# GolosChain/language-detector

Measured on AMD Instinct MI355X. Metric: docs/sec, higher is better.
Workload: dtype u8

## Files before the change

language-detector_amd/csrc/cld_wave.hip:

```cpp

namespace cld {
namespace wave {


__device__ __forceinline__ int ufl(int v) { return __builtin_amdgcn_readfirstlane(v); }
__device__ __forceinline__ uint32_t uflu(uint32_t v) { return (uint32_t)__builtin_amdgcn_readfirstlane((int)v); }
__device__ __forceinline__ uint64_t ufl64(uint64_t v) {
  return ((uint64_t)uflu((uint32_t)(v >> 32)) << 32) | uflu((uint32_t)v);
}
__device__ __forceinline__ int rdl(int v, int l) { return __builtin_amdgcn_readlane(v, l); }
__device__ __forceinline__ uint32_t rdlu(uint32_t v, int l) { return (uint32_t)__builtin_amdgcn_readlane((int)v, l); }
__device__ __forceinline__ uint64_t rdl64(uint64_t v, int l) {
  return ((uint64_t)rdlu((uint32_t)(v >> 32), l) << 32) | rdlu((uint32_t)v, l);
}


__device__ __forceinline__ void wsync() {
  __builtin_amdgcn_fence(__ATOMIC_RELEASE, "wavefront");
  __builtin_amdgcn_wave_barrier();
  __builtin_amdgcn_fence(__ATOMIC_ACQUIRE, "wavefront");
}

__device__ __forceinline__ uint64_t lanemask_lt(int lane) { return lane ? (~0ull >> (64 - lane)) : 0ull; }
__device__ __forceinline__ int below(uint64_t m) {
  return (int)__builtin_amdgcn_mbcnt_hi((uint32_t)(m >> 32), __builtin_amdgcn_mbcnt_lo((uint32_t)m, 0u));
}
__device__ __forceinline__ int lane_here() {
  int l;
  asm volatile("v_mbcnt_lo_u32_b32 %0, -1, 0\n\tv_mbcnt_hi_u32_b32 %0, -1, %0" : "=v"(l));
  return l;
}

template <int N, class V>
__device__ __forceinline__ V pick(const V (&a)[N], int r) {
  V v = a[0];
#pragma unroll
  for (int i = 1; i < N; ++i) if (r == i) v = a[i];
  return v;
}
template <int N, class V>
__device__ __forceinline__ void put_lane(V (&a)[N], int r, int l, V val) {
  const bool me = (int)__lane_id() == l;
#pragma unroll
  for (int i = 0; i < N; ++i)
    if (r == i && me) a[i] = val;
}
template <int N>
__device__ __forceinline__ void or_bit(uint64_t (&a)[N], int r, int l) {
#pragma unroll
  for (int i = 0; i < N; ++i) if (r == i) a[i] |= 1ull << l;
}

constexpr int kDppRowShr = 0x110, kDppRowBcast15 = 0x142, kDppRowBcast31 = 0x143;
template <class Op>
__device__ __forceinline__ uint32_t dpp_scan_incl(uint32_t x, uint32_t id, Op op) {
  const int xi = (int)x;
  x = op(x, (uint32_t)__builtin_amdgcn_update_dpp((int)id, xi, kDppRowShr | 1, 0xF, 0xF, false));
  x = op(x, (uint32_t)__builtin_amdgcn_update_dpp((int)id, (int)x, kDppRowShr | 2, 0xF, 0xF, false));
  x = op(x, (uint32_t)__builtin_amdgcn_update_dpp((int)id, (int)x, kDppRowShr | 4, 0xF, 0xF, false));
  x = op(x, (uint32_t)__builtin_amdgcn_update_dpp((int)id, (int)x, kDppRowShr | 8, 0xF, 0xF, false));
  x = op(x, (uint32_t)__builtin_amdgcn_update_dpp((int)id, (int)x, kDppRowBcast15, 0xA, 0xF, false));
  x = op(x, (uint32_t)__builtin_amdgcn_update_dpp((int)id, (int)x, kDppRowBcast31, 0xC, 0xF, false));
  return x;
}
struct OpAdd { __device__ uint32_t operator()(uint32_t a, uint32_t b) const { return a + b; } };
struct OpMax { __device__ uint32_t operator()(uint32_t a, uint32_t b) const { return a > b ? a : b; } };
struct OpMin { __device__ uint32_t operator()(uint32_t a, uint32_t b) const { return a < b ? a : b; } };
struct OpOr { __device__ uint32_t operator()(uint32_t a, uint32_t b) const { return a | b; } };

constexpr int kDppWaveShr1 = 0x138, kDppWaveShl1 = 0x130;
__device__ __forceinline__ uint32_t wshr1(uint32_t x, uint32_t first) {
  return (uint32_t)__builtin_amdgcn_update_dpp((int)first, (int)x, kDppWaveShr1, 0xF, 0xF, false);
}
__device__ __forceinline__ uint64_t wshr1_64(uint64_t x) {
  return ((uint64_t)wshr1((uint32_t)(x >> 32), (uint32_t)(x >> 32)) << 32) | wshr1((uint32_t)x, (uint32_t)x);
}

__device__ __forceinline__ int excl_scan(int v, int lane) {
  (void)lane;
  return (int)dpp_scan_incl((uint32_t)v, 0u, OpAdd()) - v;
}
__device__ __forceinline__ int wsum(int v) { return rdl((int)dpp_scan_incl((uint32_t)v, 0u, OpAdd()), 63); }
__device__ __forceinline__ uint32_t wmax(uint32_t v) { return rdlu(dpp_scan_incl(v, 0u, OpMax()), 63); }
__device__ __forceinline__ uint32_t wmin(uint32_t v) { return rdlu(dpp_scan_incl(v, 0xFFFFFFFFu, OpMin()), 63); }
__device__ __forceinline__ uint64_t wor64(uint64_t v) {
  const uint32_t lo = rdlu(dpp_scan_incl((uint32_t)v, 0u, OpOr()), 63);
  const uint32_t hi = rdlu(dpp_scan_incl((uint32_t)(v >> 32), 0u, OpOr()), 63);
  return ((uint64_t)hi << 32) | lo;
}

template <int CAP>
struct Cfg {
  static constexpr int DOC = CAP + 32;
  static constexpr int NM = (CAP + 63) / 64;
  static constexpr int SB = CAP + 72;
  static constexpr int LB = (SB * 3) / 2 + 64;
  static constexpr int NR = 2;
  static constexpr int NB = NR * 64;
  static constexpr int QM = ((LB + 63) / 64) * 2;
  static constexpr int NE = 160;
  static constexpr int ND = 96;
  static constexpr int NX = 160;
  static constexpr int MAXCH = NE / kChunksizeQuads + 3;
  static_assert(NB < kMaxScoringHits - 1, "a round must never reach the reference's hit cap");
  static_assert(CAP < 2048, "spans of a short document can never reach the squeeze test");
  static_assert((NE + ND + NX + 9) * kMaxLgProbScore < 65536, "tote headroom");
};

template <int CAP>
struct Smem {
  using C = Cfg<CAP>;
  uint8_t doc[C::DOC];
  uint8_t sn[C::DOC];
  uint64_t lsm[C::NM];
  uint64_t ent[C::NM];
  union alignas(16) {
    uint8_t sbuf[C::SB];
    uint16_t wsp[C::NB + 1];
    struct {
      int32_t theta[C::MAXCH];
      uint16_t st[3][C::MAXCH + 1];
    };
  };
  union alignas(16) {
    uint8_t lbuf[C::LB];
    uint32_t tote[128];
  };
  union alignas(16) {
    uint16_t nx[CAP];
    uint32_t low[CAP];
    struct {
      uint32_t be_lp[C::NE];
      uint16_t be_off[C::NE + 1];
    } e;
  } a;
  union alignas(16) {
    struct {
      uint16_t d_off[C::ND]; uint32_t d_ind[C::ND];
      uint16_t x_off[C::NX]; uint32_t x_ind[C::NX];
    };
    struct {
      uint32_t qmark[C::QM];
      uint16_t qchn[C::NB];
      uint16_t nxq[C::LB];
    };
  };
  uint16_t E[C::MAXCH];
  uint32_t lo[C::MAXCH];
  uint32_t ring[2][4];
  DocTote dt;
};

template <int NM>
__device__ __forceinline__ int find_first(const uint64_t* m, int from, int L) {
  if (from >= L) return L;
  int w = from >> 6;
  uint64_t x = ufl64(m[w]) & (~0ull << (from & 63));
  for (;;) {
    if (x) { int r = (w << 6) + __builtin_ctzll(x); return r < L ? r : L; }
    ++w;
    if (w >= NM || (w << 6) >= L) return L;
    x = ufl64(m[w]);
  }
}

__device__ __forceinline__ int cpt_index(uint32_t b0, uint32_t b1, uint32_t b2, int n) {
  if (n == 1) return (int)b0;
  if (n == 2) return 128 + (int)((b0 & 0x1F) << 6 | (b1 & 0x3F));
  return 2176 + (int)((b0 & 0x0F) << 12 | (b1 & 0x3F) << 6 | (b2 & 0x3F));
}

__device__ __forceinline__ uint32_t pack_lowered(uint64_t e) {
  const uint32_t olen = (uint32_t)(e >> 11) & 15;
  return (((e >> 10) & 1) && olen <= 3) ? (((uint32_t)(e >> 32) & 0xFFFFFFu) | olen << 24) : 0xFFFFFFFFu;
}

template <int CAP, bool PLAIN>
__device__ bool load_document(const DevTables& T, const uint8_t* __restrict__ g, int L, Smem<CAP>& s, int lane,
                              const uint8_t* __restrict__ hf, bool& lowv) {
  if constexpr (PLAIN) hf = nullptr;
  lowv = false;
  using C = Cfg<CAP>;
  static_assert(CAP == 256 && C::DOC == 288, "one aligned dword per lane covers the document");
// ... 3 lines not shown
    const uint32_t* gw = reinterpret_cast<const uint32_t*>(ga - (uintptr_t)sh);
    const int nw = (L + sh + 3) >> 2;
    const uint32_t w0 = lane < nw ? gld(gw + lane) : 0u;
    const uint32_t w64 = nw > 64 ? gld(gw + 64) : 0u;
    const uint32_t nxt = (uint32_t)__builtin_amdgcn_update_dpp((int)w64, (int)w0, kDppWaveShl1, 0xF, 0xF, false);
    const uint32_t v = sh == 0 ? w0 : __builtin_amdgcn_alignbyte(nxt, w0, (uint32_t)sh);
    const int nb = L - 4 * lane;
    const uint32_t keep = nb >= 4 ? 0xFFFFFFFFu : nb <= 0 ? 0u : (1u << (8 * nb)) - 1u;
    reinterpret_cast<uint32_t*>(s.doc)[lane] = v & keep;
    if (lane < (C::DOC - 256) / 4) reinterpret_cast<uint32_t*>(s.doc)[64 + lane] = 0u;
    if (hf) {
      for (int w = 0; w < C::NM; ++w) {
        const uint64_t m = __ballot(w * 64 + lane < L && gld(hf + w * 64 + lane) != 0);
        if (lane == 0) s.ent[w] = m;
      }
    } else if (!PLAIN && lane < C::NM) {
      s.ent[lane] = 0ull;
    }
  }
  wsync();
  DocView dv{s.doc, L};
  {
    int slow = 0, conts = 0, need = 0;
    int idx[C::NM];
#pragma unroll
    for (int w = 0; w < C::NM; ++w) idx[w] = -1;
#pragma unroll
    for (int w = 0; w < C::NM; ++w) {
      if (w * 64 >= L) break;
      const int p = w * 64 + lane;
      const uint32_t c = s.doc[p], b1 = s.doc[p + 1], b2 = s.doc[p + 2];
      const bool in = p < L;
      const bool cont = in && (c & 0xC0) == 0x80, lead = in && !cont;
      const int n = utf8_len((uint8_t)c);
      const bool bad = lead && (n > 3 || p + n > L || (n >= 2 && (b1 & 0xC0) != 0x80) || (n == 3 && (b2 & 0xC0) != 0x80));
      conts += cont ? 1 : 0;
      slow |= bad ? 1 : 0;
      const bool ok = lead && !bad;
      need += ok ? n - 1 : 0;
      idx[w] = ok ? cpt_index(c, b1, b2, n) : -1;
    }
    uint64_t ev[C::NM];
#pragma unroll
    for (int w = 0; w < C::NM; ++w) ev[w] = idx[w] >= 0 ? gld(T.cpt + idx[w]) : 0ull;
#pragma unroll
    for (int w = 0; w < C::NM; ++w) {
      if (w * 64 >= L) break;
      const int p = w * 64 + lane;
      const uint64_t e = ev[w];
      const int st = (int)((e >> 8) & 3);
      slow |= st == 3 ? 1 : 0;
      s.sn[p] = (uint8_t)e;
      s.a.low[p] = pack_lowered(e);
      const uint64_t m = __ballot(st == 1 && (e & 0xFF) != 0);
      if (lane == 0) s.lsm[w] = m;
    }
    slow |= wsum(conts - need) != 0 ? 1 : 0;
    if (__ballot(slow != 0) == 0) {
      if (lane < 4) s.sn[L + lane] = (uint8_t)script_num(T, dv, L + lane);
      wsync();
      lowv = true;
      return true;
    }
  }
  for (int p = lane; p < L + 4; p += 64) s.sn[p] = (uint8_t)script_num(T, dv, p);
  for (int p = lane; p < L; p += 64) s.a.nx[p] = (uint16_t)(p + scan_to_letter_or_special(T, dv, p, L - p));
  wsync();
  int bad = 0, conts = 0, need = 0;
  for (int p = lane; p < L; p += 64) {
    uint8_t c = s.doc[p];
    if ((c & 0xC0) == 0x80) { ++conts; continue; }
    int n = utf8_len(c);
    if (p + n > L) { bad = 1; continue; }
    for (int k = 1; k < n; ++k) bad |= ((s.doc[p + k] & 0xC0) != 0x80);
    need += n - 1;
    int np = s.a.nx[p];
    if (np != p) {
      int q = p + n;
      int want = q >= L ? L : (int)s.a.nx[q];
      bad |= (np != want);
    }
  }
  bad |= (wsum(conts) != wsum(need)) ? 1 : 0;
  if (__ballot(bad != 0)) return false;
  for (int w = 0; w < C::NM; ++w) {
    int p = w * 64 + lane;
    bool ls = false;
    if (p < L) ls = ((s.doc[p] & 0xC0) != 0x80) && s.a.nx[p] == p && s.sn[p] != 0;
    uint64_t m = __ballot(ls);
    if (lane == 0) s.lsm[w] = m;
  }
  wsync();
  return true;
}

template <int CAP>
__device__ bool stale_script_amp(const DevTables& T, Smem<CAP>& s, int L, const uint8_t* __restrict__ hf, int lane) {
  const int common = (int)T.common, inherited = (int)T.inherited;
  int hit = 0;
  for (int x = lane; x < L; x += 64) {
    if (!((s.ent[x >> 6] >> (x & 63)) & 1) || !(gld(hf + x) & 2) || (s.doc[x] & 0xC0) == 0x80) continue;
    const int sc = s.sn[x];
    if (sc == 0 || sc == common) continue;
    int b = x - 1;
    while (b > 0 && (s.doc[b] & 0xC0) == 0x80) --b;
    if (b < 0) continue;
    const int scb = s.sn[b];
    if (scb == 0 || scb == common || scb == inherited) continue;
    int a = b - 1;
    while (a > 0 && (s.doc[a] & 0xC0) == 0x80) --a;
    if (a < 0) continue;
    const int sca = s.sn[a];
    if (sca == 0 || sca == common) continue;
    hit |= (sca == inherited || (scb != sca && sc != sca)) ? 1 : 0;
  }
  return __ballot(hit != 0) != 0;
}

template <int CAP, bool PLAIN>
__device__ int next_span(const DevTables& T, Smem<CAP>& s, int L, int& next, int& ulscript, int lane) {
  lane = lane_here();
  using C = Cfg<CAP>;
  const int common = (int)T.common, inherited = (int)T.inherited;
  const int q = find_first<C::NM>(s.lsm, next, L);
  if (q >= L) { next = L; return 0; }
  const int spanscript = ufl(s.sn[q]);
  ulscript = spanscript;
  if (lane == 0) s.sbuf[0] = ' ';
  int put = 1, take = L;
  bool run = true;
  for (int w = q >> 6; w < C::NM && w * 64 < L; ++w) {
    const int x = w * 64 + lane;
    const bool valid = x >= q && x < L;
    const uint32_t c = valid ? s.doc[x] : 0u;
    const bool lead = valid && (c & 0xC0) != 0x80;
    bool brk = false, ok = false, foreign = false;
    if (lead) {
      const int sc = s.sn[x];
      if (sc != spanscript && sc != inherited) {
        if (sc == common) {
          brk = true;
        } else {
          const int xn = x + utf8_len((uint8_t)c);
          const int sc2 = (!PLAIN && xn < 64 * C::NM && ((s.ent[xn >> 6] >> (xn & 63)) & 1)) ? 0 : s.sn[xn];
          brk = sc2 != common && sc2 != spanscript;
        }
      }
      if ((s.lsm[w] >> lane) & 1) {
        if (sc == spanscript || sc == inherited) ok = true;
        else foreign = true;
      }
    }
    const uint64_t Bm = __ballot(brk), Om = __ballot(ok);
    const uint64_t evm = Bm | Om;
    const uint64_t ev_le = evm & (lane == 63 ? ~0ull : ((2ull << lane) - 1)), ev_lt = evm & lanemask_lt(lane);
    const bool inrun = ev_le ? ((Om >> (63 - __builtin_clzll(ev_le))) & 1) : run;
    const bool prev_run = ev_lt ? ((Om >> (63 - __builtin_clzll(ev_lt))) & 1) : run;
    const uint64_t Em = __ballot(foreign && (brk || !prev_run));
    const int stop = Em ? __builtin_ctzll(Em) : 64;
    const bool cp = valid && inrun && lane < stop;
    const bool sep = brk && prev_run && lane <= stop;
    const int cnt = (cp ? 1 : 0) + (sep ? 1 : 0);
    const int pos = put + excl_scan(cnt, lane);
    if (cp) s.sbuf[pos] = (uint8_t)c;
    if (sep) s.sbuf[pos] = ' ';
    put = rdl(pos + cnt, 63);
    if (stop < 64) {
      take = w * 64 + stop;
      run = false;
      break;
    }
    if (evm) run = (Om >> (63 - __builtin_clzll(evm))) & 1;
  }
  if (run) {
    if (lane == 0) s.sbuf[put] = ' ';
    ++put;
  }
  if (lane < 4) s.sbuf[put + lane] = lane < 3 ? ' ' : 0;
  next = take;
  wsync();
  return put;
}

__device__ __forceinline__ void setb(uint64_t& o, int i, uint32_t v) {
  o = (o & ~(0xFFull << (8 * i))) | ((uint64_t)(v & 0xFF) << (8 * i));
}
template <bool PIN = false>
__device__ bool lower_char_sm(const DevSM& sm_in, const uint8_t* src, int n, uint64_t& out, int& olen) {
  const DevSM sm_pin = PIN ? pinned_sm(sm_in) : DevSM{};
  const DevSM& sm = PIN ? sm_pin : sm_in;
  const int sh = (int)sm.shift;
  const int nE = 1 << sh;
  const int64_t tb0 = sm.state0;
  int64_t tb = tb0;
  out = 0; olen = 0;
  for (int i = 0; i < n; ++i) {
    const uint8_t c = src[i];
    const int e = sm8(sm, tb + c);
    if (olen >= 8) return false;
    out |= (uint64_t)c << (8 * olen);
    ++olen;
    if (e < kExitIllegalStructure) { tb = tb0 + ((int64_t)e << sh); continue; }
    switch (e) {
      case kExitReplace31:
        if (olen < 3) return false;
        olen -= 2; setb(out, olen - 1, sm8(sm, tb + c + nE * 1));
        out &= olen >= 8 ? ~0ull : ((1ull << (8 * olen)) - 1);
        break;
      case kExitReplace32:
        if (olen < 3) return false;
        olen -= 1; setb(out, olen - 2, sm8(sm, tb + c + nE * 2)); setb(out, olen - 1, sm8(sm, tb + c + nE * 1));
        out &= (1ull << (8 * olen)) - 1;
        break;
      case kExitReplace21:
// ... 48 lines not shown
    int m = utf8_len((uint8_t)b);
    if (i + m > olen) return false;
    for (int k = 1; k < m; ++k)
      if ((((uint32_t)(out >> (8 * (i + k)))) & 0xC0) != 0x80) return false;
    i += m;
  }
  return true;
}
__device__ __forceinline__ bool lower_char(const DevTables& T, const uint8_t* src, int n, uint64_t& out, int& olen) {
  return lower_char_sm(T.lower, src, n, out, olen);
}

template <int CAP>
__device__ int lower_span(const DevTables& T, Smem<CAP>& s, int text_bytes, int lane) {
  lane = lane_here();
  using C = Cfg<CAP>;
  const int ilen = text_bytes + 3;
  int obase = 0;
  int bad = 0;
  for (int w0 = 0; w0 < ilen; w0 += 64) {
    const int p = w0 + lane;
    uint64_t o = 0;
    int olen = 0;
    if (p < ilen && (s.sbuf[p] & 0xC0) != 0x80) {
      const int n = utf8_len(s.sbuf[p]);
      const uint32_t b1 = s.sbuf[p + 1], b2 = s.sbuf[p + 2];
      const bool wf = n <= 3 && (n < 2 || (b1 & 0xC0) == 0x80) && (n < 3 || (b2 & 0xC0) == 0x80);
      const uint64_t e = wf ? T.cpt[cpt_index(s.sbuf[p], b1, b2, n)] : 0ull;
      if ((e >> 10) & 1) {
        olen = (int)((e >> 11) & 15);
        o = e >> 32;
      } else if (!lower_char_sm<true>(T.lower, &s.sbuf[p], n, o, olen)) {
        bad = 1;
        olen = 0;
      }
    }
    const int pre = excl_scan(olen, lane);
    const int tot = rdl(pre + olen, 63);
    if (obase + tot + 4 > C::LB - 16) bad = 1;
    else
      for (int k = 0; k < olen; ++k) s.lbuf[obase + pre + k] = (uint8_t)(o >> (8 * k));
    obase += tot;
  }
  if (__ballot(bad != 0)) return -1;
  for (int k = lane; k < 20; k += 64) s.lbuf[obase + k] = 0;
  wsync();
  return obase - 3;
}

template <int CAP, bool PLAIN>
__device__ int span_lowered(const DevTables& T, Smem<CAP>& s, int L, int& next, int& ulscript, int lane, bool lowv) {
  lane = lane_here();
  using C = Cfg<CAP>;
  const int common = (int)T.common, inherited = (int)T.inherited;
  const int q = find_first<C::NM>(s.lsm, next, L);
  if (q >= L) { next = L; return 0; }
  const int spanscript = ufl(s.sn[q]);
  ulscript = spanscript;
  uint32_t ev[C::NM];
  if (lowv) {
#pragma unroll
    for (int w = 0; w < C::NM; ++w) ev[w] = s.a.low[w * 64 + lane];
  } else {
    int idx[C::NM];
#pragma unroll
    for (int w = 0; w < C::NM; ++w) {
      const int p = w * 64 + lane;
      const uint32_t c = s.doc[p], b1 = s.doc[p + 1], b2 = s.doc[p + 2];
      const int n = utf8_len((uint8_t)c);
      const bool wf = p >= q && p < L && (c & 0xC0) != 0x80 && n <= 3 && (n < 2 || (b1 & 0xC0) == 0x80) &&
                      (n < 3 || (b2 & 0xC0) == 0x80);
      idx[w] = wf ? cpt_index(c, b1, b2, n) : -1;
    }
    uint64_t raw[C::NM];
#pragma unroll
    for (int w = 0; w < C::NM; ++w) raw[w] = idx[w] >= 0 ? gld(T.cpt + idx[w]) : 0ull;
#pragma unroll
    for (int w = 0; w < C::NM; ++w) ev[w] = pack_lowered(raw[w]);
  }
  static_assert(C::NM == 4, "four windows");
  uint32_t e0 = ev[0], e1 = ev[1], e2 = ev[2], e3 = ev[3];
  for (int i = q >> 6; i > 0; --i) { e0 = e1; e1 = e2; e2 = e3; }
  if (lane == 0) s.lbuf[0] = ' ';
  int put = 1, take = L, bad = 0;
  bool run = true;
  for (int w = q >> 6; w < C::NM && w * 64 < L; ++w) {
    const int x = w * 64 + lane;
    const bool valid = x >= q && x < L;
    const uint32_t c = valid ? s.doc[x] : 0u;
    const bool lead = valid && (c & 0xC0) != 0x80;
    bool brk = false, ok = false, foreign = false;
    if (lead) {
      const int sc = s.sn[x];
      if (sc != spanscript && sc != inherited) {
        if (sc == common) {
          brk = true;
        } else {
          const int xn = x + utf8_len((uint8_t)c);
          const int sc2 = (!PLAIN && xn < 64 * C::NM && ((s.ent[xn >> 6] >> (xn & 63)) & 1)) ? 0 : s.sn[xn];
          brk = sc2 != common && sc2 != spanscript;
        }
      }
      if ((s.lsm[w] >> lane) & 1) {
        if (sc == spanscript || sc == inherited) ok = true;
        else foreign = true;
      }
    }
    const uint64_t Bm = __ballot(brk), Om = __ballot(ok), Fm = __ballot(foreign), Lm = __ballot(lead);
    const uint64_t evm = Bm | Om;
    const uint64_t ca = Om | ~evm;
    const uint64_t prevm = (ca + Om + (run ? 1ull : 0ull)) ^ ca ^ Om;
    const uint64_t runm = Om | (~evm & prevm);
    const uint64_t Em = Fm & (Bm | ~prevm);
    const int stop = Em ? __builtin_ctzll(Em) : 64;
    const uint64_t lt_stop = Em ? (Em & (0 - Em)) - 1 : ~0ull, le_stop = Em ? (Em ^ (Em - 1)) : ~0ull;
    const bool cl = ((Lm & runm & lt_stop) >> lane) & 1;
    const bool sep = ((Bm & prevm & le_stop) >> lane) & 1;
    const uint32_t e = e0;
    const bool low = e != 0xFFFFFFFFu;
    bad |= (cl && !low) ? 1 : 0;
    const int olen = sep ? 1 : (cl && low) ? (int)(e >> 24) : 0;
    const uint32_t o = sep ? (uint32_t)' ' : e;
    const int pos = put + excl_scan(olen, lane);
    put = rdl(pos + olen, 63);
    if (put + 8 > C::LB - 16) { bad = 1; break; }
    for (int k = 0; k < olen; ++k) s.lbuf[pos + k] = (uint8_t)(o >> (8 * k));
    if (stop < 64) {
      take = w * 64 + stop;
      run = false;
      break;
    }
    run = (runm >> 63) != 0;
    e0 = e1; e1 = e2; e2 = e3;
  }
  if (__ballot(bad != 0)) {
    const int tb = next_span<CAP, PLAIN>(T, s, L, next, ulscript, lane);
    return lower_span<CAP>(T, s, tb, lane);
  }
  if (run) {
    if (lane == 0) s.lbuf[put] = ' ';
    ++put;
  }
  if (lane < 23) s.lbuf[put + lane] = lane < 3 ? ' ' : 0;
  next = take;
  wsync();
  return put;
}

__device__ __forceinline__ uint32_t quad_hash_lds(const uint8_t* text, int p, int n) {
  const uint32_t* tw = reinterpret_cast<const uint32_t*>(text);
  const int i0 = p >> 2;
  const uint32_t sh = (uint32_t)(p & 3);
  const uint32_t x0 = tw[i0], x1 = tw[i0 + 1], x2 = tw[i0 + 2], x3 = tw[i0 + 3];
  const uint32_t y0 = __builtin_amdgcn_alignbyte(x1, x0, sh), y1 = __builtin_amdgcn_alignbyte(x2, x1, sh),
                 y2 = __builtin_amdgcn_alignbyte(x3, x2, sh);
  const uint32_t pre = (text[p - 1] == ' ' ? 0x00004444u : 0u) | (text[p + n] == ' ' ? 0x44440000u : 0u);
  const uint32_t m = (n & 3) ? (1u << (8 * (n & 3))) - 1u : 0xFFFFFFFFu;
  const uint32_t a0 = n <= 4 ? (y0 & m) : y0;
  const uint32_t w0 = (a0 ^ (a0 >> 3)) ^ pre;
  const uint32_t a1 = n <= 8 ? (y1 & m) : y1;
  const uint32_t w1 = a1 ^ (a1 << 4);
  const uint32_t a2 = y2 & m;
  const uint32_t w2 = a2 ^ (a2 << 2);
  const uint32_t r = n <= 4 ? w0 : n <= 8 ? w0 + w1 : w0 + w1 + w2;
  return n == 0 ? 0u : r;
}

template <int CAP>
__device__ __forceinline__ bool emit_base(Smem<CAP>& s, const DevTbl& bo, const DevTbl& bo2, bool kept, uint32_t ind,
                                          int off, int& eb) {
  using C = Cfg<CAP>;
  uint32_t l1 = 0, l2 = 0;
  if (kept) {
    const DevTbl* lb = &bo;
    if (ind & 0x80000000u) { lb = &bo2; ind &= ~0x80000000u; }
    if (ind < lb->size_one) {
      l1 = ind_at(*lb, ind);
    } else {
      ind += ind - lb->size_one;
      l1 = ind_at(*lb, ind); l2 = ind_at(*lb, ind + 1);
      if (l1 == 0) { l1 = l2; l2 = 0; }
    }
  }
  const uint64_t m1 = __ballot(l1 != 0), m2 = __ballot(l2 != 0);
  const int o = eb + below(m1) + below(m2);
  eb += __popcll(m1) + __popcll(m2);
  if (eb > C::NE) return false;
  if (l1) { s.a.e.be_off[o] = (uint16_t)off; s.a.e.be_lp[o] = l1; }
  if (l2) { s.a.e.be_off[o + 1] = (uint16_t)off; s.a.e.be_lp[o + 1] = l2; }
  return true;
}

template <int CAP>
__device__ int quad_hits(const DevTables& T, Smem<CAP>& s, int limit, int& nb, int& eb, int& start, int& nw, int lane) {
  lane = lane_here();
  using C = Cfg<CAP>;
  const uint8_t* text = s.lbuf;
  start = 1;
  if (text[start] == ' ') ++start;
  uint16_t* nfo = s.nxq;
  const int last = start < limit ? limit : start;
  int nws = start < limit ? 1 : 0;
  nw = 0;
  for (int w0 = start; w0 <= last; w0 += 64) {
    const int p = w0 + lane;
    const bool in = p < limit;
    const int pc = p <= last ? p : start;
    const uint32_t c0 = text[pc];
    const int a1 = pc + adv_but_space((uint8_t)c0);
    const int a2 = a1 + adv_but_space(text[a1]);
    const uint32_t c2 = text[a2];
    const int a3 = a2 + adv_but_space((uint8_t)c2);
    const int a4 = a3 + adv_but_space(text[a3]);
    const int nx = a2 + adv_space_vowel((uint8_t)c2);
    const bool fin = text[a4] == ' ' || a2 >= limit || nx >= limit;
    if (in) nfo[p] = (uint16_t)((a4 - p) | ((nx - p) << 5) | (fin ? 0x400 : 0));
    const bool sp = p <= last && c0 == ' ';
    const uint64_t m = __ballot(sp);
    if (sp) {
      const int k = nw + below(m);
      if (k <= C::NB) s.wsp[k] = (uint16_t)p;
    }
    nw += __popcll(m);
    nws += __popcll(__ballot(sp && p < limit - 1));
  }
  if (nws > C::NB || nw > C::NB) return -1;
  if (lane < C::QM) s.qmark[lane] = 0u;
  wsync();
#pragma unroll
  for (int r = 0; r < C::NR; ++r) {
    if (r * 64 >= nws) break;
    const int i = r * 64 + lane;
    if (i < nws) {
      int p = i == 0 ? start : s.wsp[i - 1] + 1;
      for (;;) {
        atomicOr(&s.qmark[p >> 5], 1u << (p & 31));
        const uint32_t f = nfo[p];
        if (f & 0x400) break;
        p += (f >> 5) & 31;
      }
    }
  }
  wsync();
  int n = 0;
  for (int w = start >> 6; w * 64 < limit; ++w) {
    const uint64_t m = ufl64(*reinterpret_cast<const uint64_t*>(&s.qmark[2 * w]));
    if ((m >> lane) & 1) {
      const int k = n + below(m);
      if (k < C::NB) s.qchn[k] = (uint16_t)(w * 64 + lane);
    }
    n += __popcll(m);
  }
  if (n > C::NB) return -1;
  wsync();
  const int end = last;
  uint32_t A = 0, B = 0;
  int base = 0;
  eb = 0;
#pragma unroll
  for (int r = 0; r < C::NR; ++r) {
    if (r * 64 >= n) break;
    const int i = r * 64 + lane;
    uint32_t hv = 0, pr = 0;
    int p = 0;
    bool hit = false;
    if (i < n) {
      p = s.qchn[i];
      hv = quad_hash_lds(text, p, (int)(nfo[p] & 31));
      uint32_t ind = 0;
      hit = quad_probe<true>(T.quad, T.quad2, hv, ind) != 0;
      pr = ind;
    }
    const uint64_t hm = __ballot(hit);
    const uint64_t hb = hm & lanemask_lt(lane);
    const int q1 = hb ? 63 - __builtin_clzll(hb) : -1;
    const uint64_t hb2 = q1 > 0 ? (hb & lanemask_lt(q1)) : 0ull;
    const int q2 = hb2 ? 63 - __builtin_clzll(hb2) : -1;
    const uint32_t h1 = (uint32_t)__shfl((int)hv, q1 < 0 ? lane : q1, 64);
    const uint32_t h2 = (uint32_t)__shfl((int)hv, q2 < 0 ? lane : q2, 64);
    const uint32_t a = q1 < 0 ? A : h1;
    const uint32_t b = q1 < 0 ? B : (q2 < 0 ? A : h2);
    const uint64_t cm = __ballot(hit && (hv == a || hv == b));
    uint64_t k = hm;
    if (cm) {
      const int f = __builtin_ctzll(cm);
      k = hm & lanemask_lt(f);
      uint32_t xA = rdlu(a, f), xB = rdlu(b, f);
      for (uint64_t rest = hm & ~lanemask_lt(f); rest; rest &= rest - 1) {
        const int l = __builtin_ctzll(rest);
        const uint32_t v = rdlu(hv, l);
        if (v == xA || v == xB) continue;
        xB = xA;
        xA = v;
        k |= 1ull << l;
      }
      A = xA;
      B = xB;
    } else if (hm) {
      const int t1 = 63 - __builtin_clzll(hm);
      const uint64_t r2 = hm & ~(1ull << t1);
      B = r2 ? rdlu(hv, 63 - __builtin_clzll(r2)) : A;
      A = rdlu(hv, t1);
    }
    if (!emit_base<CAP>(s, T.quad, T.quad2, (k >> lane) & 1, pr, p, eb)) return -1;
    base += __popcll(k);
  }
  nb = base;
  wsync();
  return end;
}

template <int CAP>
__device__ bool octa_hits(const DevTables& T, Smem<CAP>& s, int start, int nw, int& nd, int& nx, int lane) {
  lane = lane_here();
  using C = Cfg<CAP>;
  const uint8_t* text = s.lbuf;
  const uint16_t* nfo = s.nxq;
  uint64_t wh[C::NR];
  int ws[C::NR], pws[C::NR];
#pragma unroll
  for (int r = 0; r < C::NR; ++r) { wh[r] = 0; ws[r] = 0; pws[r] = 0; }
  int e1_in = start - 1, e2_in = start - 1;
#pragma unroll
  for (int r = 0; r < C::NR; ++r) {
    if (r * 64 >= nw) break;
    const int i = r * 64 + lane;
    const int e = i < nw ? (int)s.wsp[i] : 0;
    const int e1 = (int)wshr1((uint32_t)e, (uint32_t)e1_in);
    const int e2 = (int)wshr1((uint32_t)e1, (uint32_t)e2_in);
    e1_in = rdl(e, 63);
    e2_in = rdl(e1, 63);
    if (i < nw) {
      const int a = e1 + 1;
      ws[r] = a;
      pws[r] = e2 + 1;
      int we = a;
      if (a < e) {
        we += nfo[a] & 31;
        if (we < e) we += nfo[we] & 31;
      }
      wh[r] = octa_hash40(text + a, we - a);
    }
  }
  wsync();
  uint64_t keep[C::NR];
  uint32_t tlo[C::NR], thi[C::NR];
  uint64_t A = 0, B = 0;
#pragma unroll
  for (int r = 0; r < C::NR; ++r) {
    const int i = r * 64 + lane;
    const bool v = i < nw;
    const uint64_t vm = __ballot(v);
    keep[r] = 0; tlo[r] = 0; thi[r] = 0;
    if (!vm) continue;
    const int nv = __popcll(vm);
    const uint64_t w = wh[r];
    const uint64_t h1 = wshr1_64(w), h2 = wshr1_64(h1);
    const uint64_t pa = lane >= 1 ? h1 : A;
    const uint64_t pb = lane >= 2 ? h2 : (lane == 1 ? A : B);
    const uint64_t cm = __ballot(v && (w == pa || w == pb));
    uint64_t k = vm;
    uint64_t tp = pa;
    if (cm) {
      const int f = __builtin_ctzll(cm);
      k = vm & lanemask_lt(f);
      uint64_t xA = rdl64(pa, f), xB = rdl64(pb, f);
      for (int l = f; l < nv; ++l) {
        const uint64_t hv = rdl64(w, l);
        if (hv == xA || hv == xB) continue;
        if (lane == l) tp = xA;
        xB = xA;
        xA = hv;
        k |= 1ull << l;
      }
      A = xA;
      B = xB;
    } else {
      B = nv >= 2 ? rdl64(w, nv - 2) : A;
      A = rdl64(w, nv - 1);
    }
    keep[r] = k;
    tlo[r] = (uint32_t)tp;
    thi[r] = (uint32_t)(tp >> 32);
  }
  int xb = 0, db = 0;
  bool over = false;
#pragma unroll
  for (int r = 0; r < C::NR; ++r) {
    if (r * 64 >= nw) break;
    uint32_t pp = 0, xp = 0, dp = 0;
    const bool k = (keep[r] >> lane) & 1;
    if (k) {
      const uint64_t tph = ((uint64_t)thi[r] << 32) | tlo[r];
      if (tph != 0 && tph != wh[r]) pp = octa_lookup<true>(T.distinctocta, pair_hash(tph, wh[r]));
      xp = octa_lookup<true>(T.distinctocta, wh[r]);
      dp = octa_lookup<true>(T.deltaocta, wh[r]);
    }
    const uint64_t mp = __ballot(pp != 0), mx = __ballot(xp != 0), md = __ballot(dp != 0);
    const int ox = xb + below(mp) + below(mx), od = db + below(md);
    const int tx = __popcll(mp) + __popcll(mx), td = __popcll(md);
    if (xb + tx > C::NX || db + td > C::ND) { over = true; break; }
    int o = ox;
    if (pp) { s.x_off[o] = (uint16_t)pws[r]; s.x_ind[o] = pp & T.distinctocta.nkey_mask; ++o; }
    if (xp) { s.x_off[o] = (uint16_t)ws[r]; s.x_ind[o] = xp & T.distinctocta.nkey_mask; }
    if (dp) { s.d_off[od] = (uint16_t)ws[r]; s.d_ind[od] = dp & T.deltaocta.nkey_mask; }
    xb += tx; db += td;
  }
  if (over) return false;
  nd = db; nx = xb;
  wsync();
  return true;
}

template <int CAP>
__device__ int cjk_hits(const DevTables& T, Smem<CAP>& s, int limit, int& nb, int& eb, int& nd, int& nx, int lane) {
  lane = lane_here();
  using C = Cfg<CAP>;
  const uint8_t* text = s.lbuf;
  int start = 1;
  if (text[start] == ' ') ++start;
  int b = 0;
  eb = 0;
  const DevSM uni = pinned_sm(T.uni);
  uint32_t endmax = (uint32_t)start;
  for (int w0 = start; w0 < limit; w0 += 64) {
    const int p = w0 + lane;
    int prop = 0, len = 0;
    if (p < limit && (text[p] & 0xC0) != 0x80) {
      len = utf8_len(text[p]);
      prop = uni_prop_sm(uni, text + p, len);
      endmax = (uint32_t)(p + len) > endmax ? (uint32_t)(p + len) : endmax;
    }
    if (!emit_base<CAP>(s, T.compat, T.compat, prop > 0, (uint32_t)prop, p + len, eb)) return -1;
    b += __popcll(__ballot(prop > 0));
  }
  if (b > C::NB) return -1;
  const int next = (int)wmax(endmax);
  int dcount = 0, xcount = 0;
  for (int w0 = 1; w0 < next; w0 += 64) {
    const int p = w0 + lane;
    uint32_t dp = 0, xp = 0;
    if (p < next && (text[p] & 0xC0) != 0x80) {
      const int len = utf8_len(text[p]);
      const int len2 = utf8_len(text[p + len]) + len;
// ... 166 lines not shown
  }
  }
  const uint32_t seed = ((uint32_t)per_script_number_latin(T, default_language(T, ulscript)) << 8);
  const int rs = ((uint32_t)ulscript == T.latin) ? 0 : 1;
  ring_sel = rs;
  const int nboost = pri ? 2 * kMaxBoosts : kMaxBoosts;
  int ck1 = -1, ck2 = -1, cs1 = 0, cs2 = 0, cgr = 0;
  wsync();
  for (int k = 0; k < K; ++k) {
    const int seedn = k == 0 ? 1 : 0;
    const int bs = s.st[0][k], nB = s.st[0][k + 1] - bs, ds = s.st[1][k], nD = s.st[1][k + 1] - ds;
    const int xs = s.st[2][k], xe = s.st[2][k + 1], nX = xe - xs;
    const int tot = seedn + nB + nD + nX + nboost;
    auto chunk_lp = [&](int t) -> uint32_t {
      const int u0 = t - seedn, u1 = u0 - nB, u2 = u1 - nD, u3 = u2 - nX, u4 = u3 - kMaxBoosts;
      const uint32_t vb = s.a.e.be_lp[min(max(bs + u0, 0), C::NE - 1)];
      const uint32_t vd = s.d_ind[min(max(ds + u1, 0), C::ND - 1)];
      const int v = xe - kMaxBoosts + u3;
      const uint32_t vx = s.x_ind[min(max(u3 < 0 ? xs + u2 : v, 0), C::NX - 1)];
      const uint32_t vr = s.ring[rs][min(max(v + kMaxBoosts, 0), kMaxBoosts - 1)];
      const uint32_t vp = pri ? gld(pri + 4 * rs + min(max(u4, 0), kMaxBoosts - 1)) : 0u;
      const uint32_t r = u0 < 0 ? seed : u1 < 0 ? vb : u2 < 0 ? vd : u3 < 0 ? vx : u4 < 0 ? (v < 0 ? vr : vx) : vp;
      return t < tot ? r : 0u;
    };
    uint32_t lp = chunk_lp(lane);
    uint32_t e = lp ? gld(reinterpret_cast<const uint32_t*>(T.lgprob + 8 * (lp & 0xFF) + 4)) : 0u;
    reinterpret_cast<uint2*>(s.tote)[lane] = make_uint2(0, 0);
    wsync();
    uint64_t gm = 0;
    for (int t = lane;;) {
      if (lp) {
        const uint32_t k1 = (lp >> 8) & 0xFF, k2 = (lp >> 16) & 0xFF, k3 = (lp >> 24) & 0xFF;
        if (k1) { atomicAdd(&s.tote[k1 >> 1], ((e >> 8) & 0xFF) << ((k1 & 1) * 16)); gm |= 1ull << (k1 >> 2); }
        if (k2) { atomicAdd(&s.tote[k2 >> 1], ((e >> 16) & 0xFF) << ((k2 & 1) * 16)); gm |= 1ull << (k2 >> 2); }
        if (k3) { atomicAdd(&s.tote[k3 >> 1], (e >> 24) << ((k3 & 1) * 16)); gm |= 1ull << (k3 >> 2); }
      }
      t += 64;
      if (t - lane >= tot) break;
      lp = chunk_lp(t);
      e = lp ? gld(reinterpret_cast<const uint32_t*>(T.lgprob + 8 * (lp & 0xFF) + 4)) : 0u;
    }
    gm = wor64(gm);
    const int score_count = nB + seedn;
    wsync();
    if (pri) {
      const uint32_t wh = lane < 4 ? gld(pri + 8 + 4 * rs + lane) : 0u;
      if (wh > 0) {
        const uint32_t k1 = (wh >> 8) & 0xFF;
        atomicAnd(&s.tote[k1 >> 1], ~(0xFFFFu << ((k1 & 1) * 16)));
      }
      wsync();
    }
    const uint2 v2 = reinterpret_cast<const uint2*>(s.tote)[lane];
    const bool inuse = (gm >> lane) & 1;
    uint32_t cand[4] = {v2.x & 0xFFFF, v2.x >> 16, v2.y & 0xFFFF, v2.y >> 16};
    int key3[2] = {-1, -1};
    uint32_t sc3[2] = {0, 0};
#pragma unroll
    for (int r = 0; r < 2; ++r) {
      uint32_t best = 0;
#pragma unroll
      for (int i = 0; i < 4; ++i) {
        const int key = lane * 4 + i;
        const bool taken = key == key3[0];
        const uint32_t comp = (inuse && !taken) ? ((cand[i] + 1) << 8) | (uint32_t)(255 - key) : 0u;
        best = comp > best ? comp : best;
      }
      best = wmax(best);
      if (best) { key3[r] = 255 - (int)(best & 0xFF); sc3[r] = (best >> 8) - 1; }
    }
    if (lane == k) {
      ck1 = key3[0]; ck2 = key3[1];
      cs1 = key3[0] >= 0 ? (int)sc3[0] : 0;
      cs2 = key3[1] >= 0 ? (int)sc3[1] : 0;
      cgr = score_count;
    }
    wsync();
  }
  const int nsum = K < kMaxSummaries ? K : kMaxSummaries;
  if constexpr (DEFER) {
    if (nrec + nsum > kTailRecs) return false;
    if (lane < nsum) {
      const uint32_t lo_k = s.lo[lane];
      const int lo = lo_k == 0xFFFFFFFFu ? dummy_off : (int)lo_k;
      int hi = dummy_off;
      if (lane + 1 < K && s.lo[lane + 1] != 0xFFFFFFFFu) hi = (int)s.lo[lane + 1];
      rec[1 + nrec + lane] = tail_chunk_record(ck1, ck2, cs1, cs2, cgr, lo, hi, ulscript);
    }
    nrec += nsum;
  } else {
  int sum_lang = 0, sum_bytes = 0, sum_rel = 0;
  if (lane < K) {
    const uint32_t lo_k = s.lo[lane];
    const int lo = lo_k == 0xFFFFFFFFu ? dummy_off : (int)lo_k;
    int hi = dummy_off;
    if (lane + 1 < K && s.lo[lane + 1] != 0xFFFFFFFFu) hi = (int)s.lo[lane + 1];
    const uint64_t* kt = T.keytab + 256 * (uint32_t)ulscript;
    const uint64_t i1 = gld(kt + (uint8_t)ck1), i2 = gld(kt + (uint8_t)ck2);
    const int lang1 = (int)(i1 & 0xFFFF);
    const int len = hi - lo;
    int actual = 0;
    if (len > 0) actual = (int)((uint32_t)cs1 << 10) / len;
    const int expected = (int16_t)(uint16_t)(i1 >> 32);
    const uint16_t bytes = (uint16_t)len, grams = (uint16_t)cgr;
    const uint16_t s1 = (uint16_t)cs1, s2 = (uint16_t)cs2;
    int rd = (uint8_t)reliability_delta(s1, s2, grams);
    const int c1 = (int)((i1 >> 16) & 0xFFFF);
    if (c1 != 0 && c1 == (int)((i2 >> 16) & 0xFFFF)) rd = 100;
    const int rsc = (uint8_t)reliability_expected(actual, expected);
    sum_lang = (uint16_t)lang1; sum_bytes = bytes; sum_rel = rd < rsc ? rd : rsc;
    cs1 = s1;
  }
  for (int k = 0; k < nsum; ++k) {
    const int l1 = rdl(sum_lang, k), by = rdl(sum_bytes, k), sc = rdl(cs1, k), rl = rdl(sum_rel, k);
    dt_add_wave(s.dt, l1, by, sc, rl, lane);
  }
  }
  if (lane == 0) {
    uint32_t r4[4];
    for (int i = 0; i < 4; ++i) {
      const int u = ex + i;
      r4[i] = u < 4 ? s.ring[rs][u] : s.x_ind[u - 4];
    }
    for (int i = 0; i < 4; ++i) s.ring[rs][i] = r4[i];
  }
  wsync();
  return true;
}

struct SlotRegs {
  uint32_t key;
  int val, sc, rl;
};
__device__ __forceinline__ SlotRegs load_slots(const DocTote& dt, int lane) {
  const bool in = lane < 24;
  const int j = in ? lane : 0;
  SlotRegs r;
  r.key = in ? dt.key[j] : kUnusedKey;
  r.val = in ? dt.value[j] : -1;
  r.sc = in ? dt.score[j] : 0;
  r.rl = in ? dt.rel[j] : 0;
  return r;
}

__device__ __forceinline__ void sort3_regs(SlotRegs& r, int lane) {
  const bool in = lane < 24;
  if (r.key == kUnusedKey) r.val = -1;
#pragma unroll
  for (int p = 0; p < 3; ++p) {
    const uint32_t m = dpp_scan_incl((in && lane >= p) ? (uint32_t)r.val ^ 0x80000000u : 0u, 0u, OpMax());
    const int ex = (int)(wshr1(m, 0u) ^ 0x80000000u);
    const uint64_t R = __ballot(in && lane > p && r.val > ex);
    if (R) {
      const uint64_t below = R & lanemask_lt(lane);
      const int src = lane == p ? 63 - __builtin_clzll(R)
                    : ((R >> lane) & 1) ? (below ? 63 - __builtin_clzll(below) : p) : lane;
      r.key = (uint32_t)__shfl((int)r.key, src, 64);
      r.val = __shfl(r.val, src, 64);
      r.sc = __shfl(r.sc, src, 64);
      r.rl = __shfl(r.rl, src, 64);
    }
  }
}

struct NoMove {
  __device__ __forceinline__ void operator()(int, int) const {}
};
template <class Mv = NoMove>
__device__ __forceinline__ void refine_close_pairs_regs(const DevTables& T, SlotRegs& r, int lane, Mv&& mv = Mv{}) {
  int cs = lane < 24 ? close_set(T, (int)r.key) : 0;
  uint64_t todo = __ballot(cs != 0);
  while (todo) {
    const int s = __builtin_ctzll(todo);
    todo &= todo - 1;
    const int css = rdl(cs, s);
    if (css == 0) continue;
    const uint64_t mm = __ballot(lane > s && cs == css);
    if (!mm) continue;
    const int s2 = __builtin_ctzll(mm);
    const bool s_from = rdl(r.val, s) < rdl(r.val, s2);
    const int from = s_from ? s : s2, to = s_from ? s2 : s;
    const int fv = rdl(r.val, from), fs = rdl(r.sc, from), fr = rdl(r.rl, from);
    mv(rdl((int)r.key, from), rdl((int)r.key, to));
    if (lane == to) { r.val += fv; r.sc += fs; r.rl += fr; }
    if (lane == from) { r.key = kUnusedKey; r.sc = 0; r.rl = 0; cs = 0; }
  }
}

__device__ __forceinline__ void remove_unreliable_regs(const DevTables& T, SlotRegs& r, uint64_t todo, int lane) {
  const int unk = (int)T.unknown_lang;
  while (todo) {
    const int s = __builtin_ctzll(todo);
    todo &= todo - 1;
    const int lang = rdl((int)r.key, s);
    if (lang == kUnusedKey) continue;
    const int bytes = rdl(r.val, s), reli = rdl(r.rl, s);
    if (bytes == 0) continue;
    const int rp = reli / bytes;
    if (rp >= 41) continue;
    int alt = unk;
    if ((uint32_t)lang <= T.hawaiian && (uint32_t)lang < T.n_closest) alt = gld(T.closest + lang);
    if (alt == unk) continue;
    const uint64_t am = __ballot(lane < 24 && (int)r.key == alt);
    if (!am) continue;
    const int as = __builtin_ctzll(am);
    const int bytes2 = rdl(r.val, as), reli2 = rdl(r.rl, as);
    if (bytes2 == 0) continue;
    const int rp2 = reli2 / bytes2;
    int to = as, from = s;
// ... 195 lines not shown
```

Before: 286.0 million.

## Use mask-based wave predicates and precompute per-byte quad classes in LDS

Replaces per-lane boolean logic with wave-wide 64-bit mask arithmetic, using inverse_ballot to read per-lane bits and splitting compound ballots into ANDed ballots. Span event detection in next_span and span_lowered is factored into a shared helper built on masks. A per-byte class table (advance length, space/vowel and space flags) is precomputed in LDS before quad hashing, so the four-step chain walk reads the table instead of recomputing UTF-8 advances. This removes VALU work and divergent branches per byte, at the cost of an extra LDS pass, a wave sync, and reusing the nx/low union region for the class table.

```diff
diff --git a/language-detector_amd/csrc/cld_wave.hip b/language-detector_amd/csrc/cld_wave.hip
--- a/language-detector_amd/csrc/cld_wave.hip
+++ b/language-detector_amd/csrc/cld_wave.hip
@@ -25,6 +25,8 @@
 __device__ __forceinline__ int below(uint64_t m) {
   return (int)__builtin_amdgcn_mbcnt_hi((uint32_t)(m >> 32), __builtin_amdgcn_mbcnt_lo((uint32_t)m, 0u));
 }
+__device__ __forceinline__ bool lane_bit(uint64_t m) { return __builtin_amdgcn_inverse_ballot_w64(m); }
+__device__ __forceinline__ uint64_t first_lanes(int n) { return n >= 64 ? ~0ull : n <= 0 ? 0ull : (1ull << n) - 1; }
 __device__ __forceinline__ int lane_here() {
   int l;
   asm volatile("v_mbcnt_lo_u32_b32 %0, -1, 0\n\tv_mbcnt_hi_u32_b32 %0, -1, %0" : "=v"(l));
@@ -129,6 +131,7 @@
   union alignas(16) {
     uint16_t nx[CAP];
     uint32_t low[CAP];
+    uint8_t qcls[C::LB];
     struct {
       uint32_t be_lp[C::NE];
       uint16_t be_off[C::NE + 1];
@@ -238,7 +241,7 @@
       slow |= st == 3 ? 1 : 0;
       s.sn[p] = (uint8_t)e;
       s.a.low[p] = pack_lowered(e);
-      const uint64_t m = __ballot(st == 1 && (e & 0xFF) != 0);
+      const uint64_t m = __ballot(st == 1) & __ballot((uint8_t)e != 0);
       if (lane == 0) s.lsm[w] = m;
     }
     slow |= wsum(conts - need) != 0 ? 1 : 0;
@@ -304,10 +307,34 @@
 }
 
 template <int CAP, bool PLAIN>
+__device__ __forceinline__ void span_events(const DevTables& T, const Smem<CAP>& s, int w, int q, int L, int lane,
+                                            int spanscript, uint32_t& c, uint64_t& validm, uint64_t& Lm, uint64_t& Bm,
+                                            uint64_t& Om, uint64_t& Fm) {
+  using C = Cfg<CAP>;
+  const int common = (int)T.common, inherited = (int)T.inherited;
+  const int x = w * 64 + lane;
+  const int lo = q - w * 64 > 0 ? q - w * 64 : 0, hi = L - w * 64;
+  validm = (hi >= 64 ? ~0ull : (1ull << hi) - 1) & (~0ull << lo);
+  c = s.doc[x];
+  const int sc = s.sn[x];
+  Lm = validm & __ballot((c & 0xC0) != 0x80);
+  const uint64_t ownm = __ballot(sc == spanscript) | __ballot(sc == inherited), comm = __ballot(sc == common);
+  uint64_t lookm = 0;
+  if (Lm & ~ownm & ~comm) {
+    const int xn = x + utf8_len((uint8_t)c);
+    const int sc2 = (!PLAIN && xn < 64 * C::NM && ((s.ent[xn >> 6] >> (xn & 63)) & 1)) ? 0 : s.sn[xn];
+    lookm = ~(__ballot(sc2 == common) | __ballot(sc2 == spanscript));
+  }
+  Bm = Lm & ~ownm & (comm | lookm);
+  const uint64_t Sm = ufl64(s.lsm[w]);
+  Om = Lm & Sm & ownm;
+  Fm = Lm & Sm & ~ownm;
+}
+
+template <int CAP, bool PLAIN>
 __device__ int next_span(const DevTables& T, Smem<CAP>& s, int L, int& next, int& ulscript, int lane) {
   lane = lane_here();
   using C = Cfg<CAP>;
-  const int common = (int)T.common, inherited = (int)T.inherited;
   const int q = find_first<C::NM>(s.lsm, next, L);
   if (q >= L) { next = L; return 0; }
   const int spanscript = ufl(s.sn[q]);
@@ -316,36 +343,18 @@
   int put = 1, take = L;
   bool run = true;
   for (int w = q >> 6; w < C::NM && w * 64 < L; ++w) {
-    const int x = w * 64 + lane;
-    const bool valid = x >= q && x < L;
-    const uint32_t c = valid ? s.doc[x] : 0u;
-    const bool lead = valid && (c & 0xC0) != 0x80;
-    bool brk = false, ok = false, foreign = false;
-    if (lead) {
-      const int sc = s.sn[x];
-      if (sc != spanscript && sc != inherited) {
-        if (sc == common) {
-          brk = true;
-        } else {
-          const int xn = x + utf8_len((uint8_t)c);
-          const int sc2 = (!PLAIN && xn < 64 * C::NM && ((s.ent[xn >> 6] >> (xn & 63)) & 1)) ? 0 : s.sn[xn];
-          brk = sc2 != common && sc2 != spanscript;
-        }
-      }
-      if ((s.lsm[w] >> lane) & 1) {
-        if (sc == spanscript || sc == inherited) ok = true;
-        else foreign = true;
-      }
-    }
-    const uint64_t Bm = __ballot(brk), Om = __ballot(ok);
+    uint32_t c;
+    uint64_t validm, Lm, Bm, Om, Fm;
+    span_events<CAP, PLAIN>(T, s, w, q, L, lane, spanscript, c, validm, Lm, Bm, Om, Fm);
     const uint64_t evm = Bm | Om;
     const uint64_t ev_le = evm & (lane == 63 ? ~0ull : ((2ull << lane) - 1)), ev_lt = evm & lanemask_lt(lane);
     const bool inrun = ev_le ? ((Om >> (63 - __builtin_clzll(ev_le))) & 1) : run;
     const bool prev_run = ev_lt ? ((Om >> (63 - __builtin_clzll(ev_lt))) & 1) : run;
-    const uint64_t Em = __ballot(foreign && (brk || !prev_run));
+    const uint64_t prevm = __ballot(prev_run);
+    const uint64_t Em = Fm & (Bm | ~prevm);
     const int stop = Em ? __builtin_ctzll(Em) : 64;
-    const bool cp = valid && inrun && lane < stop;
-    const bool sep = brk && prev_run && lane <= stop;
+    const bool cp = lane_bit(validm) && inrun && lane < stop;
+    const bool sep = lane_bit(Bm & prevm) && lane <= stop;
     const int cnt = (cp ? 1 : 0) + (sep ? 1 : 0);
     const int pos = put + excl_scan(cnt, lane);
     if (cp) s.sbuf[pos] = (uint8_t)c;
@@ -500,7 +509,6 @@
 __device__ int span_lowered(const DevTables& T, Smem<CAP>& s, int L, int& next, int& ulscript, int lane, bool lowv) {
   lane = lane_here();
   using C = Cfg<CAP>;
-  const int common = (int)T.common, inherited = (int)T.inherited;
   const int q = find_first<C::NM>(s.lsm, next, L);
   if (q >= L) { next = L; return 0; }
   const int spanscript = ufl(s.sn[q]);
@@ -530,31 +538,13 @@
   uint32_t e0 = ev[0], e1 = ev[1], e2 = ev[2], e3 = ev[3];
   for (int i = q >> 6; i > 0; --i) { e0 = e1; e1 = e2; e2 = e3; }
   if (lane == 0) s.lbuf[0] = ' ';
-  int put = 1, take = L, bad = 0;
+  int put = 1, take = L;
+  bool bad = false;
   bool run = true;
   for (int w = q >> 6; w < C::NM && w * 64 < L; ++w) {
-    const int x = w * 64 + lane;
-    const bool valid = x >= q && x < L;
-    const uint32_t c = valid ? s.doc[x] : 0u;
-    const bool lead = valid && (c & 0xC0) != 0x80;
-    bool brk = false, ok = false, foreign = false;
-    if (lead) {
-      const int sc = s.sn[x];
-      if (sc != spanscript && sc != inherited) {
-        if (sc == common) {
-          brk = true;
-        } else {
-          const int xn = x + utf8_len((uint8_t)c);
-          const int sc2 = (!PLAIN && xn < 64 * C::NM && ((s.ent[xn >> 6] >> (xn & 63)) & 1)) ? 0 : s.sn[xn];
-          brk = sc2 != common && sc2 != spanscript;
-        }
-      }
-      if ((s.lsm[w] >> lane) & 1) {
-        if (sc == spanscript || sc == inherited) ok = true;
-        else foreign = true;
-      }
-    }
-    const uint64_t Bm = __ballot(brk), Om = __ballot(ok), Fm = __ballot(foreign), Lm = __ballot(lead);
+    uint32_t c;
+    uint64_t validm, Lm, Bm, Om, Fm;
+    span_events<CAP, PLAIN>(T, s, w, q, L, lane, spanscript, c, validm, Lm, Bm, Om, Fm);
     const uint64_t evm = Bm | Om;
     const uint64_t ca = Om | ~evm;
     const uint64_t prevm = (ca + Om + (run ? 1ull : 0ull)) ^ ca ^ Om;
@@ -562,17 +552,24 @@
     const uint64_t Em = Fm & (Bm | ~prevm);
     const int stop = Em ? __builtin_ctzll(Em) : 64;
     const uint64_t lt_stop = Em ? (Em & (0 - Em)) - 1 : ~0ull, le_stop = Em ? (Em ^ (Em - 1)) : ~0ull;
-    const bool cl = ((Lm & runm & lt_stop) >> lane) & 1;
-    const bool sep = ((Bm & prevm & le_stop) >> lane) & 1;
+    const uint64_t clm = Lm & runm & lt_stop;
+    const uint64_t sepm = Bm & prevm & le_stop;
     const uint32_t e = e0;
-    const bool low = e != 0xFFFFFFFFu;
-    bad |= (cl && !low) ? 1 : 0;
-    const int olen = sep ? 1 : (cl && low) ? (int)(e >> 24) : 0;
+    const uint64_t lowm = __ballot(e != 0xFFFFFFFFu);
+    bad |= (clm & ~lowm) != 0;
+    const bool sep = lane_bit(sepm);
+    const int olen = sep ? 1 : lane_bit(clm & lowm) ? (int)(e >> 24) : 0;
     const uint32_t o = sep ? (uint32_t)' ' : e;
     const int pos = put + excl_scan(olen, lane);
     put = rdl(pos + olen, 63);
-    if (put + 8 > C::LB - 16) { bad = 1; break; }
-    for (int k = 0; k < olen; ++k) s.lbuf[pos + k] = (uint8_t)(o >> (8 * k));
+    if (put + 8 > C::LB - 16) { bad = true; break; }
+    if (olen > 0) {
+      s.lbuf[pos] = (uint8_t)o;
+      if (olen > 1) {
+        s.lbuf[pos + 1] = (uint8_t)(o >> 8);
+        if (olen > 2) s.lbuf[pos + 2] = (uint8_t)(o >> 16);
+      }
+    }
     if (stop < 64) {
       take = w * 64 + stop;
       run = false;
@@ -581,7 +578,7 @@
     run = (runm >> 63) != 0;
     e0 = e1; e1 = e2; e2 = e3;
   }
-  if (__ballot(bad != 0)) {
+  if (bad) {
     const int tb = next_span<CAP, PLAIN>(T, s, L, next, ulscript, lane);
     return lower_span<CAP>(T, s, tb, lane);
   }
@@ -614,6 +611,15 @@
   return n == 0 ? 0u : r;
 }
 
+__device__ __forceinline__ uint32_t quad_class(uint32_t c) {
+  constexpr uint32_t kVowels = 1u << 1 | 1u << 5 | 1u << 9 | 1u << 15 | 1u << 21;
+  const int ones = __builtin_clz(~(c << 24));
+  const bool low = c <= 0x20;
+  const uint32_t adv = low ? 0u : (uint32_t)min(max(ones, 1), 4);
+  const bool sv = low || ones == 1 || ((c & 0xC0) == 0x40 && ((kVowels >> (c & 31)) & 1));
+  return adv | (sv ? 8u : 0u) | (c == ' ' ? 16u : 0u);
+}
+
 template <int CAP>
 __device__ __forceinline__ bool emit_base(Smem<CAP>& s, const DevTbl& bo, const DevTbl& bo2, bool kept, uint32_t ind,
                                           int off, int& eb) {
@@ -650,27 +656,33 @@
   const int last = start < limit ? limit : start;
   int nws = start < limit ? 1 : 0;
   nw = 0;
+  constexpr int kQuadPad = 22;
+  uint8_t* cls = s.a.qcls;
+  for (int w0 = start; w0 <= last + kQuadPad; w0 += 64) {
+    const int pc = lane_bit(first_lanes(last + kQuadPad - w0 + 1)) ? w0 + lane : start;
+    cls[pc] = (uint8_t)quad_class(text[pc]);
+  }
+  wsync();
   for (int w0 = start; w0 <= last; w0 += 64) {
     const int p = w0 + lane;
-    const bool in = p < limit;
-    const int pc = p <= last ? p : start;
-    const uint32_t c0 = text[pc];
-    const int a1 = pc + adv_but_space((uint8_t)c0);
-    const int a2 = a1 + adv_but_space(text[a1]);
-    const uint32_t c2 = text[a2];
-    const int a3 = a2 + adv_but_space((uint8_t)c2);
-    const int a4 = a3 + adv_but_space(text[a3]);
-    const int nx = a2 + adv_space_vowel((uint8_t)c2);
-    const bool fin = text[a4] == ' ' || a2 >= limit || nx >= limit;
-    if (in) nfo[p] = (uint16_t)((a4 - p) | ((nx - p) << 5) | (fin ? 0x400 : 0));
-    const bool sp = p <= last && c0 == ' ';
-    const uint64_t m = __ballot(sp);
-    if (sp) {
-      const int k = nw + below(m);
+    const uint64_t lastm = first_lanes(last - w0 + 1), inm = first_lanes(limit - w0);
+    const int pc = lane_bit(lastm) ? p : start;
+    const uint32_t k0 = cls[pc];
+    const int a1 = pc + (int)(k0 & 7);
+    const int a2 = a1 + (cls[a1] & 7);
+    const uint32_t k2 = cls[a2];
+    const int a3 = a2 + (int)(k2 & 7);
+    const int a4 = a3 + (cls[a3] & 7);
+    const int nx = a2 + (int)((k2 >> 3) & 1);
+    const uint64_t spm = lastm & __ballot(k0 >= 16);
+    const uint64_t finm = __ballot(cls[a4] >= 16) | __ballot(a2 >= limit) | __ballot(nx >= limit);
+    if (lane_bit(inm)) nfo[p] = (uint16_t)((a4 - p) | ((nx - p) << 5) | (lane_bit(finm) ? 0x400 : 0));
+    if (lane_bit(spm)) {
+      const int k = nw + below(spm);
       if (k <= C::NB) s.wsp[k] = (uint16_t)p;
     }
-    nw += __popcll(m);
-    nws += __popcll(__ballot(sp && p < limit - 1));
+    nw += __popcll(spm);
+    nws += __popcll(spm & first_lanes(limit - 1 - w0));
   }
   if (nws > C::NB || nw > C::NB) return -1;
   if (lane < C::QM) s.qmark[lane] = 0u;
@@ -693,7 +705,7 @@
   int n = 0;
   for (int w = start >> 6; w * 64 < limit; ++w) {
     const uint64_t m = ufl64(*reinterpret_cast<const uint64_t*>(&s.qmark[2 * w]));
-    if ((m >> lane) & 1) {
+    if (lane_bit(m)) {
       const int k = n + below(m);
       if (k < C::NB) s.qchn[k] = (uint16_t)(w * 64 + lane);
     }
@@ -728,7 +740,7 @@
     const uint32_t h2 = (uint32_t)__shfl((int)hv, q2 < 0 ? lane : q2, 64);
     const uint32_t a = q1 < 0 ? A : h1;
     const uint32_t b = q1 < 0 ? B : (q2 < 0 ? A : h2);
-    const uint64_t cm = __ballot(hit && (hv == a || hv == b));
+    const uint64_t cm = hm & (__ballot(hv == a) | __ballot(hv == b));
     uint64_t k = hm;
     if (cm) {
       const int f = __builtin_ctzll(cm);
@@ -750,7 +762,7 @@
       B = r2 ? rdlu(hv, 63 - __builtin_clzll(r2)) : A;
       A = rdlu(hv, t1);
     }
-    if (!emit_base<CAP>(s, T.quad, T.quad2, (k >> lane) & 1, pr, p, eb)) return -1;
+    if (!emit_base<CAP>(s, T.quad, T.quad2, lane_bit(k), pr, p, eb)) return -1;
     base += __popcll(k);
   }
   nb = base;
@@ -806,7 +818,7 @@
     const uint64_t h1 = wshr1_64(w), h2 = wshr1_64(h1);
     const uint64_t pa = lane >= 1 ? h1 : A;
     const uint64_t pb = lane >= 2 ? h2 : (lane == 1 ? A : B);
-    const uint64_t cm = __ballot(v && (w == pa || w == pb));
+    const uint64_t cm = vm & (__ballot(w == pa) | __ballot(w == pb));
     uint64_t k = vm;
     uint64_t tp = pa;
     if (cm) {
@@ -837,7 +849,7 @@
   for (int r = 0; r < C::NR; ++r) {
     if (r * 64 >= nw) break;
     uint32_t pp = 0, xp = 0, dp = 0;
-    const bool k = (keep[r] >> lane) & 1;
+    const bool k = lane_bit(keep[r]);
     if (k) {
       const uint64_t tph = ((uint64_t)thi[r] << 32) | tlo[r];
       if (tph != 0 && tph != wh[r]) pp = octa_lookup<true>(T.distinctocta, pair_hash(tph, wh[r]));
@@ -1110,7 +1122,7 @@
       wsync();
     }
     const uint2 v2 = reinterpret_cast<const uint2*>(s.tote)[lane];
-    const bool inuse = (gm >> lane) & 1;
+    const bool inuse = lane_bit(gm);
     uint32_t cand[4] = {v2.x & 0xFFFF, v2.x >> 16, v2.y & 0xFFFF, v2.y >> 16};
     int key3[2] = {-1, -1};
     uint32_t sc3[2] = {0, 0};
@@ -1212,7 +1224,7 @@
     if (R) {
       const uint64_t below = R & lanemask_lt(lane);
       const int src = lane == p ? 63 - __builtin_clzll(R)
-                    : ((R >> lane) & 1) ? (below ? 63 - __builtin_clzll(below) : p) : lane;
+                    : lane_bit(R) ? (below ? 63 - __builtin_clzll(below) : p) : lane;
       r.key = (uint32_t)__shfl((int)r.key, src, 64);
       r.val = __shfl(r.val, src, 64);
       r.sc = __shfl(r.sc, src, 64);
```

After: 293.6 million, median of 6. 2.7% higher.
